# noegroup/bgflow

Measured on AMD Instinct MI355X. Metric: flow samples/s (fwd+log|detJ|) at batch 2^20, higher is better.
Workload: dtype f32 (split-f16 conditioner GEMMs: hi+lo f16 operand pairs, f32 accumulate)

## Files before the change

### bgflow_amd/csrc/bgk_fused2.hip

```cpp
#include "bgk_common.h"
#include "bgk_fused2.h"

#ifndef BGK_V2_SAVE
#define BGK_V2_SAVE 0
#endif
#if BGK_V2_SAVE
#include "bgk_mfma_h2.h"
#include "bgk_rqs_vjp.h"
#define coupling_rqs_dense_h2v2_kernel coupling_rqs_dense_h2v2_train_kernel
#endif
#ifndef BGK_V2_BF16
#define BGK_V2_BF16 0
#endif
#if BGK_V2_BF16
#define coupling_rqs_dense_h2v2_kernel coupling_rqs_dense_h2v2_bf16_kernel
typedef short s16x8 __attribute__((ext_vector_type(8)));
#endif
#ifndef BGK_V2_AFFTRAIN
#define BGK_V2_AFFTRAIN 0
#endif
#if BGK_V2_AFFTRAIN
#define coupling_affine_dense_v2_kernel coupling_affine_dense_v2_train_kernel
#endif
constexpr int NPROD = BGK_V2_BF16 ? 1 : 3;
// ... 150 lines not shown
    template <int E0, int E1>
    __device__ __forceinline__ void events() {
        if constexpr (E0 < E1) {
            event<E0>();
            events<E0 + 1, E1>();
        }
    }
    template <int HK, int NH>
    __device__ __forceinline__ void hook() {
        constexpr int e0 = (HK * NEV) / NH, e1 = ((HK + 1) * NEV) / NH;
        if constexpr (e0 < e1) events<e0, e1>();
    }
};
struct NoLive {
    template <int HK, int NH> __device__ __forceinline__ void hook() {}
};

template <int NT>
struct LiveTM {
    static constexpr int LPT = KS + 1;
    static constexpr int NLS = LPT * NT;
    static constexpr int EPT = 3 * KS + 1;
    static constexpr int NEV = EPT * NT;
    static constexpr int tile_of(int i) { return NT == 4 ? (i == 0 ? 1 : (i == 1 ? 3 : (i == 2 ? 0 : 2))) : (i == 0 ? 1 : 0); }
    f32x16 (&out)[4];
    const BFrag& b;
    const uint4* W;
    unsigned voff;
    TFrag (&ring)[RD];
    __amdgpu_buffer_rsrc_t rs;

    template <int BLK>
    __device__ __forceinline__ u32x4 blk() {
        return __builtin_amdgcn_raw_buffer_load_b128(rs, voff + ((BLK * 1024) & 4095), (BLK * 1024) & ~4095, 0);
    }
    template <int L>
    __device__ __forceinline__ void load() {
        if constexpr (L < NLS) {
            constexpr int s = L % LPT, m = tile_of(L / LPT);
            if constexpr (s < KS) {
                ring[L % RD].hi = blk<(s * 4 + m) * 2>();
                ring[L % RD].lo = blk<(s * 4 + m) * 2 + 1>();
            } else {
                ring[L % RD].hi = blk<KS * 4 * 2 + m>();
            }
        }
    }
    template <int L0, int L1>
    __device__ __forceinline__ void loads() {
        if constexpr (L0 < L1) { load<L0>(); loads<L0 + 1, L1>(); }
    }
    __device__ __forceinline__ void start() {
        __builtin_amdgcn_sched_barrier(0);
        rs = __builtin_amdgcn_make_buffer_rsrc((void*)W, 0, 0x7fffffff, 0x00020000);
        loads<0, RD>();
        __builtin_amdgcn_sched_barrier(0);
    }
    template <int E>
    __device__ __forceinline__ void event() {
        __builtin_amdgcn_sched_barrier(0);
        if constexpr (E < NEV) {
            constexpr int i = E / EPT, e = E % EPT, m = tile_of(i);
            if constexpr (e < 3 * KS) {
                constexpr int s = e / 3, p = e % 3, L = i * LPT + s;
                const TFrag& f = ring[L % RD];
                const h16x8 a = __builtin_bit_cast(h16x8, p == 0 ? f.lo : f.hi);
                const h16x8 bb = p == 1 ? b.lo[s] : b.hi[s];
                if constexpr (s == 0 && p == 0) {
                    const f32x16 z = {0.f, 0.f, 0.f, 0.f, 0.f, 0.f, 0.f, 0.f, 0.f, 0.f, 0.f, 0.f, 0.f, 0.f, 0.f, 0.f};
                    out[m] = __builtin_amdgcn_mfma_f32_32x32x16_f16(a, bb, z, 0, 0, 0);
                } else {
                    out[m] = __builtin_amdgcn_mfma_f32_32x32x16_f16(a, bb, out[m], 0, 0, 0);
                }
                if constexpr (p == 2) load<L + RD>();
            } else {
                constexpr int L = i * LPT + KS;
                const h16x8 one2 = {(_Float16)1.0f, (_Float16)1.0f, 0, 0, 0, 0, 0, 0};
                out[m] = __builtin_amdgcn_mfma_f32_32x32x16_f16(__builtin_bit_cast(h16x8, ring[L % RD].hi), one2, out[m], 0, 0, 0);
                load<L + RD>();
            }
        }
        __builtin_amdgcn_sched_barrier(0);
    }
    template <int E0, int E1>
    __device__ __forceinline__ void events() {
        if constexpr (E0 < E1) {
            event<E0>();
            events<E0 + 1, E1>();
        }
    }
    template <int HK, int NH>
    __device__ __forceinline__ void hook() {
        constexpr int e0 = (HK * NEV) / NH, e1 = ((HK + 1) * NEV) / NH;
        if constexpr (e0 < e1) events<e0, e1>();
    }
};

template <class G, int BASE, int NH>
struct Hooks {
    G& g;
    template <int I> __device__ __forceinline__ void at() { g.template hook<BASE + I, NH>(); }
};

template <int ACT, int T, int P, class H>
__device__ __forceinline__ void act_split_pair(H& hk, const f32x16& t, float c, BFrag& bf) {
    constexpr int r = 2 * P;
    float a0, a1;
    if constexpr (ACT == 2) {
        a0 = t[r] * c; a1 = t[r + 1] * c;
        hk.template at<3 * P>();
        a0 = a0 > 0.0f ? a0 : 0.0f; a1 = a1 > 0.0f ? a1 : 0.0f;
        hk.template at<3 * P + 1>();
    } else {
        constexpr float kk = ACT == 1 ? -1.44269504088896341f : 2.88539008177792681f;
        const float ck = c * kk, rc = 1.0f / c;
        const float e0 = __builtin_amdgcn_exp2f(t[r] * ck), e1 = __builtin_amdgcn_exp2f(t[r + 1] * ck);
        hk.template at<3 * P>();
        if constexpr (ACT == 1) {
            const float q0 = __builtin_amdgcn_rcpf(__builtin_fmaf(e0, rc, rc)), q1 = __builtin_amdgcn_rcpf(__builtin_fmaf(e1, rc, rc));
            a0 = t[r] * q0; a1 = t[r + 1] * q1;
        } else {
            const float q0 = __builtin_amdgcn_rcpf(1.0f + e0), q1 = __builtin_amdgcn_rcpf(1.0f + e1);
            a0 = 1.0f - 2.0f * q0; a1 = 1.0f - 2.0f * q1;
        }
        hk.template at<3 * P + 1>();
    }
    constexpr int s = 2 * T + (r >> 3), e = r & 7;
#if BGK_V2_BF16
    typedef __bf16 bf2v __attribute__((ext_vector_type(2)));
    typedef float f2v __attribute__((ext_vector_type(2)));
    typedef _Float16 h2v __attribute__((ext_vector_type(2)));
    const bf2v pb = __builtin_convertvector((f2v){a0, a1}, bf2v);
    const h2v ph = __builtin_bit_cast(h2v, pb);
    bf.hi[s][e] = ph[0]; bf.hi[s][e + 1] = ph[1];
#else
    unsigned uh, ul;
    asm("v_cvt_pk_f16_f32 %0, %1, %2" : "=v"(uh) : "v"(a0), "v"(a1));
    asm("v_fma_mixlo_f16 %0, %1, -1.0, %2 op_sel:[0,0,0] op_sel_hi:[1,0,0]" : "=v"(ul) : "v"(uh), "v"(a0));
    asm("v_fma_mixhi_f16 %0, %1, -1.0, %2 op_sel:[1,0,0] op_sel_hi:[1,0,0]" : "+v"(ul) : "v"(uh), "v"(a1));
    typedef _Float16 h2v __attribute__((ext_vector_type(2)));
    const h2v ph = __builtin_bit_cast(h2v, uh), pl = __builtin_bit_cast(h2v, ul);
    bf.hi[s][e] = ph[0]; bf.hi[s][e + 1] = ph[1];
    bf.lo[s][e] = pl[0]; bf.lo[s][e + 1] = pl[1];
#endif
    hk.template at<3 * P + 2>();
}
template <int ACT, int T, class H>
__device__ __forceinline__ void act_split_tile(H hk, const f32x16& t, float c, BFrag& bf) {
    act_split_pair<ACT, T, 0>(hk, t, c, bf); act_split_pair<ACT, T, 1>(hk, t, c, bf);
    act_split_pair<ACT, T, 2>(hk, t, c, bf); act_split_pair<ACT, T, 3>(hk, t, c, bf);
    act_split_pair<ACT, T, 4>(hk, t, c, bf); act_split_pair<ACT, T, 5>(hk, t, c, bf);
    act_split_pair<ACT, T, 6>(hk, t, c, bf); act_split_pair<ACT, T, 7>(hk, t, c, bf);
}

struct SpK { float kL, kz, c2; };

__device__ __forceinline__ float fdiv_hw(float n, float d) {
    const float r = __builtin_amdgcn_rcpf(d);
    const float q = n * r;
    return __builtin_fmaf(__builtin_fmaf(-d, q, n), r, q);
}

template <bool KARG> struct ScSrc;
template <> struct ScSrc<true> {
    kargs_t ka;
    __device__ __forceinline__ ScSrc(const V2Args&) { ka = (kargs_t)__builtin_amdgcn_kernarg_segment_ptr(); asm volatile("" : "+s"(ka)); }
    __device__ __forceinline__ const __attribute__((address_space(4))) SpC& get() const { return ka->sc; }
};
template <> struct ScSrc<false> {
    const V2Args& a;
    __device__ __forceinline__ ScSrc(const V2Args& a_) : a(a_) {}
    __device__ __forceinline__ const SpC& get() const { return a.sc; }
};

template <int INV, class H>
__device__ __forceinline__ float rqs_fast(H hk, float x, const float (&va)[KB], const float (&vb)[KB], const float* ps, int pst, bool circ,
                                          const V2Args& a, const SpK& k, float* lad, int* bin, int* oob) {
    const ScSrc<(BGK_V2_KARG == 2 ? INV != 0 : BGK_V2_KARG != 0)> scs(a);
#define SC scs.get()
    *oob = (x < SC.left) | (x > SC.right);
    x = __builtin_amdgcn_fmed3f(x, SC.left, SC.right);
    float mA = __builtin_fmaxf(__builtin_fmaxf(va[0], va[1]), va[2]);
    mA = __builtin_fmaxf(__builtin_fmaxf(mA, va[3]), va[4]);
    mA = __builtin_fmaxf(__builtin_fmaxf(mA, va[5]), va[6]);
    mA = __builtin_fmaxf(mA, va[7]);
    const float nmA = -(mA * k.kL);
    hk.template at<0>();
    float E[KB];
    E[0] = __builtin_amdgcn_exp2f(__builtin_fmaf(va[0], k.kL, nmA));
    E[1] = __builtin_amdgcn_exp2f(__builtin_fmaf(va[1], k.kL, nmA));
    E[2] = __builtin_amdgcn_exp2f(__builtin_fmaf(va[2], k.kL, nmA));
    hk.template at<1>();
    E[3] = __builtin_amdgcn_exp2f(__builtin_fmaf(va[3], k.kL, nmA));
    E[4] = __builtin_amdgcn_exp2f(__builtin_fmaf(va[4], k.kL, nmA));
    E[5] = __builtin_amdgcn_exp2f(__builtin_fmaf(va[5], k.kL, nmA));
    hk.template at<2>();
    E[6] = __builtin_amdgcn_exp2f(__builtin_fmaf(va[6], k.kL, nmA));
    E[7] = __builtin_amdgcn_exp2f(__builtin_fmaf(va[7], k.kL, nmA));
    E[1] += E[0]; E[2] += E[1];
    hk.template at<3>();
    E[3] += E[2]; E[4] += E[3]; E[5] += E[4]; E[6] += E[5]; E[7] += E[6];
    hk.template at<4>();
    const float gA = SC.sa.gnum * bgk_rcp_refined(E[7]);
    float kn[7];
    kn[0] = __builtin_fmaf(E[0], gA, SC.sa.kc[0]);
    kn[1] = __builtin_fmaf(E[1], gA, SC.sa.kc[1]);
    hk.template at<5>();
    kn[2] = __builtin_fmaf(E[2], gA, SC.sa.kc[2]);
    kn[3] = __builtin_fmaf(E[3], gA, SC.sa.kc[3]);
    kn[4] = __builtin_fmaf(E[4], gA, SC.sa.kc[4]);
    kn[5] = __builtin_fmaf(E[5], gA, SC.sa.kc[5]);
    kn[6] = __builtin_fmaf(E[6], gA, SC.sa.kc[6]);
    hk.template at<6>();
    float low_a = SC.sa.low, high_a = SC.sa.high;
    asm volatile("" : "+s"(low_a), "+s"(high_a));
#pragma unroll
    for (int i = 0; i < 7; ++i) asm volatile("" : "+v"(kn[i]));
    const bool g3 = x >= kn[3];
    hk.template at<7>();
    float w0 = g3 ? kn[3] : low_a, w1 = g3 ? kn[4] : kn[0], w2 = g3 ? kn[5] : kn[1], w3 = g3 ? kn[6] : kn[2];
    hk.template at<8>();
    float w4 = g3 ? high_a : kn[3];
    const bool gm = x >= w2;
    const float v0 = gm ? w2 : w0, v1 = gm ? w3 : w1, v2 = gm ? w4 : w2;
    hk.template at<9>();
    const bool gl = x >= v1;
    const float lo = gl ? v1 : v0, hi = gl ? v2 : v1;
    float idxf = g3 ? 4.0f : 0.0f;
    hk.template at<10>();
    idxf += gm ? 2.0f : 0.0f;
    idxf += gl ? 1.0f : 0.0f;
    const int idx = (int)idxf;
    *bin = idx;
    hk.template at<11>();
    const int j1 = circ ? ((idx + 1) & 7) : (idx + 1);
    const float s_lo = ps[idx * pst], s_hi = ps[j1 * pst];
    const float A_i = hi - lo;
    float mB = __builtin_fmaxf(__builtin_fmaxf(vb[0], vb[1]), vb[2]);
    hk.template at<12>();
    mB = __builtin_fmaxf(__builtin_fmaxf(mB, vb[3]), vb[4]);
    mB = __builtin_fmaxf(__builtin_fmaxf(mB, vb[5]), vb[6]);
    mB = __builtin_fmaxf(mB, vb[7]);
    const float nmB = -(mB * k.kL);
    float F[KB];
    F[0] = __builtin_amdgcn_exp2f(__builtin_fmaf(vb[0], k.kL, nmB));
    hk.template at<13>();
    F[1] = __builtin_amdgcn_exp2f(__builtin_fmaf(vb[1], k.kL, nmB));
    F[2] = __builtin_amdgcn_exp2f(__builtin_fmaf(vb[2], k.kL, nmB));
    F[3] = __builtin_amdgcn_exp2f(__builtin_fmaf(vb[3], k.kL, nmB));
    hk.template at<14>();
    F[4] = __builtin_amdgcn_exp2f(__builtin_fmaf(vb[4], k.kL, nmB));
    F[5] = __builtin_amdgcn_exp2f(__builtin_fmaf(vb[5], k.kL, nmB));
    F[6] = __builtin_amdgcn_exp2f(__builtin_fmaf(vb[6], k.kL, nmB));
    hk.template at<15>();
    F[7] = __builtin_amdgcn_exp2f(__builtin_fmaf(vb[7], k.kL, nmB));
    F[1] += F[0]; F[2] += F[1]; F[3] += F[2];
    hk.template at<16>();
    F[4] += F[3]; F[5] += F[4]; F[6] += F[5]; F[7] += F[6];
    const float rB = __builtin_amdgcn_rcpf(F[7]);
    hk.template at<17>();
    const float gB = SC.sb.gnum * __builtin_fmaf(__builtin_fmaf(-F[7], rB, 1.0f), rB, rB);
    const float f0 = g3 ? F[3] : 0.0f, f1 = g3 ? F[4] : F[0], f2 = g3 ? F[5] : F[1];
    hk.template at<18>();
    const float f3 = g3 ? F[6] : F[2], f4 = g3 ? F[7] : F[3];
    const float u0 = gm ? f2 : f0, u1 = gm ? f3 : f1, u2 = gm ? f4 : f2;
    hk.template at<19>();
    const float Flo = gl ? u1 : u0;
    float Fhi = gl ? u2 : u1;
    hk.template at<20>();
    const float cb = __builtin_fmaf(idxf, SC.sb.dstep, SC.sb.low);
    hk.template at<21>();
    const float b_i = __builtin_fmaf(Flo, gB, cb);
    float b_ip1 = __builtin_fmaf(Fhi, gB, cb + SC.sb.dstep);
    float top_b = SC.sb.high;
    asm volatile("" : "+s"(top_b));
    b_ip1 = (g3 && gm && gl) ? top_b : b_ip1;
    const float B_i = b_ip1 - b_i;
    const float z0 = s_lo * k.kz;
    hk.template at<22>();
    const float ez0 = __builtin_amdgcn_exp2f(z0);
    float lg0 = __builtin_amdgcn_logf(1.0f + ez0);
    asm volatile("" : "+v"(lg0));
    const float sm0 = ez0 * __builtin_fmaf(ez0, -0.5f, 1.0f) * 1.44269504088896341f;
    hk.template at<23>();
    float l0 = (ez0 < 2.44140625e-4f ? sm0 : lg0) * SC.kout;
    asm volatile("" : "+v"(l0));
    l0 = z0 > 28.8539008177792681f ? s_lo * k.c2 : l0;
    const float d_i = SC.min_d + l0;
    const float z1 = s_hi * k.kz;
    hk.template at<24>();
    const float ez1 = __builtin_amdgcn_exp2f(z1);
    float lg1 = __builtin_amdgcn_logf(1.0f + ez1);
    asm volatile("" : "+v"(lg1));
    const float sm1 = ez1 * __builtin_fmaf(ez1, -0.5f, 1.0f) * 1.44269504088896341f;
    hk.template at<25>();
    float l1 = (ez1 < 2.44140625e-4f ? sm1 : lg1) * SC.kout;
    asm volatile("" : "+v"(l1));
    l1 = z1 > 28.8539008177792681f ? s_hi * k.c2 : l1;
    const float d_ip1 = SC.min_d + l1;
    float cw_i, W_i, ch_i, H_i;
    if (INV) { cw_i = lo; W_i = A_i; ch_i = b_i; H_i = B_i; }
    else { ch_i = lo; H_i = A_i; cw_i = b_i; W_i = B_i; }
    hk.template at<26>();
    const float delta = fdiv_hw(H_i, W_i);
    const float S = d_i + d_ip1 - 2.0f * delta;
    hk.template at<27>();
// ... 170 lines not shown
    s_y[valid ? j * a.ys + dim : 32 * a.ys + j] = o;
    oob_local += (valid && j < rows) ? oob : 0;
    bins[IT] = bin;
    lad = valid ? lad : 0.0f;
    float l0 = lad, l1 = lad;
    asm volatile("s_nop 1\n\tv_permlane32_swap_b32 %0, %1" : "+v"(l0), "+v"(l1));
    run += l0;
    run += l1;
}

template <int INV, int NT>
__device__ __forceinline__ void chunk_piped_reg(const V2Args& a, const SpK& k, float* s_p, float* s_y, int c, int hh, int j, int rows,
                                                float& run, int& oob_local, int (&bins)[3], f32x16 (&h)[4], const BFrag& bf,
                                                TFrag (&ring)[RD], unsigned voff) {
    LiveTM<NT> g{h, bf, a.A2 + (size_t)(c + 1) * GBLK * 64, voff, ring};
    g.start();
    slab_to_lds(h, s_p, hh, j);
    __builtin_amdgcn_sched_barrier(0);
    spline_slot_reg<INV, 0, 3 * EH>(g, a, k, h[0], s_p, s_y, c, DPC, hh, j, rows, run, oob_local, bins);
    spline_slot_reg<INV, 1, 3 * EH>(g, a, k, h[2], s_p, s_y, c, DPC, hh, j, rows, run, oob_local, bins);
    spline_slot_reg<INV, 2, 3 * EH>(g, a, k, h[2], s_p, s_y, c, DPC, hh, j, rows, run, oob_local, bins);
}

typedef const __attribute__((address_space(1))) void* gvp_t;
typedef __attribute__((address_space(3))) void* lvp_t;
__device__ __forceinline__ void dma_tile32(float* dst, const float* __restrict__ src, int n, int valid, int lane) {
    for (int c = 0; c < n; c += 256) {
        const int e = c + lane * 4;
        if (e + 3 < valid) __builtin_amdgcn_global_load_lds((gvp_t)(src + e), (lvp_t)(dst + c), 16, 0, 0);
    }
    if (valid & 3) {
        const int edge = valid & ~3;
        if (lane < (valid & 3)) __builtin_amdgcn_global_load_lds((gvp_t)(src + edge + lane), (lvp_t)(dst + edge), 4, 0, 0);
    }
}

__device__ __forceinline__ void v2_sincos2pi(float x, float* s, float* c) {
    const float f = __builtin_amdgcn_fractf(x);
    *s = __builtin_amdgcn_sinf(f);
    *c = __builtin_amdgcn_cosf(f);
}

struct StageTiles { int d_c, periodic, nfs, ys, stage, y_dma, d; uint32_t magic_d; int rows, lane; };

__device__ __forceinline__ void stage_issue(const StageTiles& t, const CondSegs& cs, int64_t b0, const float* y_t, float* s_p, float* s_y) {
    if (t.y_dma) dma_tile32(s_y, y_t, 32 * t.d, t.rows * t.d, t.lane);
    if (t.stage == 1) dma_tile32(s_p, cs.ptr[0] + b0 * cs.ld[0], 32 * t.d_c, t.rows * t.d_c, t.lane);
    else if (t.stage == 2) dma_tile32(s_p + 32 * t.nfs, cs.ptr[0] + b0 * cs.ld[0], 32 * t.d_c, t.rows * t.d_c, t.lane);
}

#ifndef BGK_V2_SB
#define BGK_V2_SB 8
#endif
template <class KA>
__device__ __forceinline__ void stage_finish(const StageTiles& t, const CondSegs& cs, int64_t b0, const float* y_t, int ldy32,
                                             float* s_p, float* s_y, float y_fill) {
    constexpr int SB = BGK_V2_SB;
    const int lane = t.lane, rows = t.rows, d = t.d, nfs = t.nfs, n_y = 32 * t.d;
    if (!t.y_dma) {
        for (int base = 0; base < n_y; base += 64 * SB) {
            float vy[SB];
#pragma unroll
            for (int u = 0; u < SB; ++u) {
                const int i = base + u * 64 + lane;
                const int r = (int)(__umul24((unsigned)i, t.magic_d) >> 20), c = i - (int)__umul24((unsigned)r, (unsigned)d);
                vy[u] = (i < n_y && r < rows) ? y_t[(int)__umul24((unsigned)r, (unsigned)ldy32) + c] : y_fill;
            }
#pragma unroll
            for (int u = 0; u < SB; ++u) {
                const int i = base + u * 64 + lane;
                const int r = (int)(__umul24((unsigned)i, t.magic_d) >> 20), c = i - (int)__umul24((unsigned)r, (unsigned)d);
                if (i < n_y) s_y[(int)__umul24((unsigned)r, (unsigned)t.ys) + c] = vy[u];
            }
        }
    }
    if (t.stage == 0) {
        typedef const __attribute__((address_space(4))) KA* ka_t;
        const ka_t kseg = (ka_t)__builtin_amdgcn_kernarg_segment_ptr();
        for (int sg = 0; sg < cs.n; ++sg) {
            const float* cond_t = kseg->cs.ptr[sg] + b0 * kseg->cs.ld[sg];
            const int ldc32 = (int)kseg->cs.ld[sg], w_c = kseg->cs.w[sg], n_c = 32 * w_c, col0 = kseg->cs.off[sg];
            const uint32_t magic_c = kseg->cs.magic[sg];
            for (int base = 0; base < n_c; base += 64 * SB) {
                float vc[SB];
#pragma unroll
                for (int u = 0; u < SB; ++u) {
                    const int i = base + u * 64 + lane;
                    const int r = (int)(__umul24((unsigned)i, magic_c) >> 20), c = i - (int)__umul24((unsigned)r, (unsigned)w_c);
                    vc[u] = (i < n_c && r < rows) ? cond_t[(int)__umul24((unsigned)r, (unsigned)ldc32) + c] : 0.0f;
                }
#pragma unroll
                for (int u = 0; u < SB; ++u) {
                    const int i = base + u * 64 + lane;
                    const int r = (int)(__umul24((unsigned)i, magic_c) >> 20), c = i - (int)__umul24((unsigned)r, (unsigned)w_c);
                    if (i < n_c) {
                        float* f = s_p + (int)__umul24((unsigned)r, (unsigned)nfs) + col0 + c;
                        if (t.periodic) {
                            float sv, cv;
                            v2_sincos2pi(vc[u], &sv, &cv);
                            f[0] = cv;
                            f[t.d_c] = sv;
                        } else {
                            f[0] = vc[u];
                        }
                    }
                }
            }
        }
    }
    asm volatile("s_waitcnt vmcnt(0)" ::: "memory");
    __builtin_amdgcn_fence(__ATOMIC_ACQ_REL, "wavefront");
    __builtin_amdgcn_wave_barrier();
    if (t.stage == 2) {
        const float* raw = s_p + 32 * nfs;
        const uint32_t magic_c = cs.magic[0];
        for (int i = lane; i < 32 * t.d_c; i += 64) {
            const int r = (int)(__umul24((unsigned)i, magic_c) >> 20), c = i - (int)__umul24((unsigned)r, (unsigned)t.d_c);
            float sv, cv;
            v2_sincos2pi(raw[i], &sv, &cv);
            float* f = s_p + (int)__umul24((unsigned)r, (unsigned)nfs) + c;
            f[0] = cv;
            f[t.d_c] = sv;
        }
    }
    if (t.stage != 1) {
        __builtin_amdgcn_fence(__ATOMIC_ACQ_REL, "wavefront");
        __builtin_amdgcn_wave_barrier();
    }
}

__device__ __forceinline__ void store_tile32(float* out_t, int ldo32, const float* s_y, int ys, int d, uint32_t magic_d, int rows, int lane, int lin) {
    const int n = rows * d;
    if (lin) {
        for (int i = lane * 4; i + 3 < n; i += 256) *reinterpret_cast<float4*>(out_t + i) = *reinterpret_cast<const float4*>(s_y + i);
        if (lane < (n & 3)) out_t[(n & ~3) + lane] = s_y[(n & ~3) + lane];
    } else {
        for (int i = lane; i < n; i += 64) {
            const int r = (int)(__umul24((unsigned)i, magic_d) >> 20), cc = i - (int)__umul24((unsigned)r, (unsigned)d);
            out_t[(int)__umul24((unsigned)r, (unsigned)ldo32) + cc] = s_y[(int)__umul24((unsigned)r, (unsigned)ys) + cc];
        }
    }
}

struct L0Frag { uint4 v[4][2]; };
__device__ __forceinline__ void l0_request(L0Frag& f, const uint4* A0, int s, int lane) {
#pragma unroll
    for (int m = 0; m < 4; ++m) {
        f.v[m][0] = A0[((s * 4 + m) * 2 + 0) * 64 + lane];
#if !BGK_V2_BF16
        f.v[m][1] = A0[((s * 4 + m) * 2 + 1) * 64 + lane];
#endif
    }
}
__device__ __forceinline__ void l0_step(f32x16 (&h)[4], const L0Frag& fr, const float* f, bool last, int rel0) {
    float v[8];
#pragma unroll
    for (int e = 0; e < 8; ++e) v[e] = f[e];
    if (last) {
#pragma unroll
        for (int e = 0; e < 8; ++e) v[e] = rel0 + e == 0 ? 1.0f : (rel0 + e > 0 ? 0.0f : v[e]);
    }
#if BGK_V2_BF16
    s16x8 bb;
#pragma unroll
    for (int e = 0; e < 8; ++e) bb[e] = __builtin_bit_cast(short, (__bf16)v[e]);
#pragma unroll
    for (int m = 0; m < 4; ++m)
        h[m] = __builtin_amdgcn_mfma_f32_32x32x16_bf16(__builtin_bit_cast(s16x8, fr.v[m][0]), bb, h[m], 0, 0, 0);
#else
    h16x8 bhi, blo;
#pragma unroll
    for (int e = 0; e < 8; ++e) {
        const float c = v[e];
        const _Float16 hv = (_Float16)c;
        bhi[e] = hv;
        blo[e] = (_Float16)(c - (float)hv);
    }
#pragma unroll
    for (int m = 0; m < 4; ++m) h[m] = __builtin_amdgcn_mfma_f32_32x32x16_f16(__builtin_bit_cast(h16x8, fr.v[m][1]), bhi, h[m], 0, 0, 0);
#pragma unroll
    for (int m = 0; m < 4; ++m) h[m] = __builtin_amdgcn_mfma_f32_32x32x16_f16(__builtin_bit_cast(h16x8, fr.v[m][0]), blo, h[m], 0, 0, 0);
#pragma unroll
    for (int m = 0; m < 4; ++m) h[m] = __builtin_amdgcn_mfma_f32_32x32x16_f16(__builtin_bit_cast(h16x8, fr.v[m][0]), bhi, h[m], 0, 0, 0);
#endif
}

template <int ACT, int INV, bool SAVEP = true, bool REGP = false>
__global__ __launch_bounds__(FTHREADS, 2) void coupling_rqs_dense_h2v2_kernel(V2Args a) {
    static_assert(!REGP || (!BGK_V2_SAVE && !BGK_V2_BF16), "row order 2 belongs to the split-f16 inference instance");
    if (a.cs_dev) { a.c0 = a.cs_dev[1]; a.c1 = a.cs_dev[3]; a.c2 = a.cs_dev[5]; }
    asm volatile("s_setreg_imm32_b32 hwreg(HW_REG_MODE, 23, 1), 1");
    extern __shared__ __attribute__((aligned(16))) float smem[];
    const int wave = REGP ? __builtin_amdgcn_readfirstlane((int)(threadIdx.x >> 6)) : (int)(threadIdx.x >> 6);
    float* s_p = smem + (size_t)wave * a.lds_per_wave;
    float* s_y = s_p + (REGP ? a.p_floats : 128 * ST);
    const int d = a.d;
    const int64_t n_tiles = (a.B + 31) / 32;
    const int64_t tile = (int64_t)blockIdx.x * FW + wave;
    if (tile >= n_tiles) return;
    const SpK k{a.c2 * 1.44269504088896341f, a.c2 * a.sc.beta * 1.44269504088896341f, a.c2};
    const int n_in = a.periodic ? 2 * a.d_c : a.d_c;
    const int ldy32 = (int)a.ldy, ldo32 = (int)a.ldo;
    const int n_y = 32 * d;

  {
    const int lane = (int)threadIdx.x & 63, j = lane & 31, hh = lane >> 5;
    const unsigned voff = (unsigned)lane * 16u;
    const int64_t b0 = tile * 32;
    const int rows = (int)((a.B - b0) < 32 ? (a.B - b0) : 32);
    const float* y_t = a.y + b0 * a.ldy;
    float* out_t = a.out + b0 * a.ldo;
    V2_TS(0);

    const int nfs = a.nfs, ys = a.ys;
    const StageTiles stg{a.d_c, a.periodic, nfs, ys, a.stage, a.y_dma, d, a.magic_d, rows, lane};
    stage_issue(stg, a.cs, b0, y_t, s_p, s_y);
    f32x16 h[4], acc[4];
    TFrag ring[RD];
    BFrag bf;
    L0Frag fa, fb;
    l0_request(fa, a.A0, 0, lane);
    Live<4> g1{acc, bf, a.A1, voff, ring};
    g1.start();
    V2_TS(12);
    stage_finish<V2Args>(stg, a.cs, b0, y_t, ldy32, s_p, s_y, 0.5f);
    V2_TS(1);

#pragma unroll
    for (int m = 0; m < 4; ++m)
#pragma unroll
        for (int r = 0; r < 16; ++r) h[m][r] = 0.0f;
    {
        const float* frow = s_p + j * nfs + 8 * hh;
        const int rel0 = 16 * (a.S0 - 1) + 8 * hh - n_in;
        for (int s = 0; s < a.S0; s += 2) {
            if (s + 1 < a.S0) l0_request(fb, a.A0, s + 1, lane);
            l0_step(h, fa, frow + 16 * s, s + 1 == a.S0, rel0);
            if (s + 1 < a.S0) {
                if (s + 2 < a.S0) l0_request(fa, a.A0, s + 2, lane);
                l0_step(h, fb, frow + 16 * (s + 1), s + 2 == a.S0, rel0);
            }
        }
    }

    V2_TS(2);
    {
        Live<4>& g = g1;
#if BGK_V2_SAVE
#pragma unroll
        for (int m = 0; m < 4; ++m)
#pragma unroll
            for (int r = 0; r < 16; ++r) h[m][r] *= a.c0;
        h2_store_rows128(h, a.z0, s_p, b0, rows, lane);
        const float c0_act = 1.0f;
#else
        const float c0_act = a.c0;
#endif
        NoLive none;
        act_split_tile<ACT, 0>(Hooks<NoLive, 0, 1>{none}, h[0], c0_act, bf);
        __builtin_amdgcn_sched_barrier(0);
        V2_TS(14);
        act_split_tile<ACT, 1>(Hooks<Live<4>, 0, 100>{g}, h[1], c0_act, bf);
        act_split_tile<ACT, 2>(Hooks<Live<4>, 24, 100>{g}, h[2], c0_act, bf);
        act_split_tile<ACT, 3>(Hooks<Live<4>, 48, 100>{g}, h[3], c0_act, bf);
        __builtin_amdgcn_sched_barrier(0);
        V2_TS(15);
        g.template events<(72 * Live<4>::NEV) / 100, Live<4>::NEV>();
    }

    V2_TS(3);
    float run = 0.0f;
    int oob_local = 0;
    {
        Live<4> g{h, bf, a.A2, voff, ring};
        g.start();
#if BGK_V2_SAVE
#pragma unroll
        for (int m = 0; m < 4; ++m)
#pragma unroll
            for (int r = 0; r < 16; ++r) acc[m][r] *= a.c1;
        h2_store_rows128(acc, a.z1, s_p, b0, rows, lane);
        const float c1_act = 1.0f;
#else
        const float c1_act = a.c1;
#endif
        NoLive none;
        act_split_tile<ACT, 0>(Hooks<NoLive, 0, 1>{none}, acc[0], c1_act, bf);
        __builtin_amdgcn_sched_barrier(0);
        act_split_tile<ACT, 1>(Hooks<Live<4>, 0, 100>{g}, acc[1], c1_act, bf);
        act_split_tile<ACT, 2>(Hooks<Live<4>, 24, 100>{g}, acc[2], c1_act, bf);
        act_split_tile<ACT, 3>(Hooks<Live<4>, 48, 100>{g}, acc[3], c1_act, bf);
        __builtin_amdgcn_sched_barrier(0);
        g.template events<(72 * Live<4>::NEV) / 100, Live<4>::NEV>();
    }
    V2_TS(4);
    for (int c = 0; c < a.n_chunks; ++c) {
        int bins[3] = {0, 0, 0};
        const int nd = (d - c * DPC) < DPC ? (d - c * DPC) : DPC;
        if constexpr (REGP) {
            if (c + 2 < a.n_chunks || (c + 2 == a.n_chunks && a.last_tiles > 2)) {
                chunk_piped_reg<INV, 4>(a, k, s_p, s_y, c, hh, j, rows, run, oob_local, bins, h, bf, ring, voff);
            } else if (c + 2 == a.n_chunks) {
                chunk_piped_reg<INV, 2>(a, k, s_p, s_y, c, hh, j, rows, run, oob_local, bins, h, bf, ring, voff);
            } else {
                NoLive none;
                slab_to_lds(h, s_p, hh, j);
                spline_slot_reg<INV, 0, 1>(none, a, k, h[0], s_p, s_y, c, nd, hh, j, rows, run, oob_local, bins);
                if (nd > 2) spline_slot_reg<INV, 1, 1>(none, a, k, h[2], s_p, s_y, c, nd, hh, j, rows, run, oob_local, bins);
                if (nd > 4) spline_slot_reg<INV, 2, 1>(none, a, k, h[2], s_p, s_y, c, nd, hh, j, rows, run, oob_local, bins);
            }
        } else
        if (c + 2 < a.n_chunks || (c + 2 == a.n_chunks && a.last_tiles > 2)) {
            chunk_piped<INV, 4, SAVEP>(a, k, s_p, s_y, c, hh, j, rows, run, oob_local, bins, h, bf, ring, voff, b0);
        } else if (c + 2 == a.n_chunks) {
            chunk_piped<INV, 2, SAVEP>(a, k, s_p, s_y, c, hh, j, rows, run, oob_local, bins, h, bf, ring, voff, b0);
        } else {
            NoLive none;
            chunk_to_lds(h, s_p, hh, j);
#if BGK_V2_SAVE
            if constexpr (SAVEP) save_chunk_params(a, s_p, c, lane, b0, rows);
#endif
            spline_slot<INV, 0, 1>(none, a, k, s_p, s_y, c, nd, hh, j, rows, run, oob_local, bins);
            if (nd > 2) spline_slot<INV, 1, 1>(none, a, k, s_p, s_y, c, nd, hh, j, rows, run, oob_local, bins);
            if (nd > 4) spline_slot<INV, 2, 1>(none, a, k, s_p, s_y, c, nd, hh, j, rows, run, oob_local, bins);
        }
#if BGK_V2_TS
        V2_TS(5 + c);
#else
        if (a.bin_idx) {
#pragma unroll
            for (int it = 0; it < 3; ++it) {
                const int q = 2 * it + hh;
                if (q < nd && j < rows) a.bin_idx[(b0 + j) * d + c * DPC + q] = bins[it];
            }
        }
#endif
        __builtin_amdgcn_fence(__ATOMIC_ACQ_REL, "wavefront");
        __builtin_amdgcn_wave_barrier();
    }
    int lane_e = lane;
    if constexpr (REGP) {
        int zero = 0;
        asm volatile("" : "+v"(zero));
        lane_e = (int)__builtin_amdgcn_mbcnt_hi(~0u, __builtin_amdgcn_mbcnt_lo(~0u, (unsigned)zero));
    }
    if ((lane_e >> 5) == 0 && (lane_e & 31) < rows) {
        if (a.accumulate) a.dlogp[b0 + (lane_e & 31)] += run; else a.dlogp[b0 + (lane_e & 31)] = run;
    }
    store_tile32(out_t, ldo32, s_y, ys, d, a.magic_d, rows, lane_e, a.out_lin);
    if (a.oob_count && __builtin_amdgcn_ballot_w64(oob_local != 0)) {
        for (int off = 32; off > 0; off >>= 1) oob_local += __shfl_xor(oob_local, off);
        if (lane_e == 0) atomicAdd(a.oob_count, oob_local);
    }
    V2_TS(5 + a.n_chunks);
  }
}

struct TilePlan { int nfs, ys, stage, y_dma, out_lin; };
TilePlan plan_tiles(const CondSegs& cs, int d_c, int periodic, const float* y, int64_t ldy, const float* out, int64_t ldo, int d, int tile_floats) {
    const int n_in = periodic ? 2 * d_c : d_c;
    const auto dma_ok = [](const float* p, int64_t ld, int w) { return ld == w && ((uintptr_t)p & 15) == 0 && (w & 7) != 0; };
    TilePlan t;
    t.y_dma = dma_ok(y, ldy, d) ? 1 : 0;
    t.ys = t.y_dma ? d : (d | 1);
    t.out_lin = (t.y_dma && ldo == d && ((uintptr_t)out & 15) == 0) ? 1 : 0;
    const bool c_dma = cs.n == 1 && dma_ok(cs.ptr[0], cs.ld[0], d_c);
    t.stage = (c_dma && !periodic) ? 1 : ((c_dma && periodic && 32 * ((n_in | 1) + d_c) <= tile_floats) ? 2 : 0);
    t.nfs = t.stage == 1 ? d_c : (n_in | 1);
    return t;
}

SetK make_set(double low, double high, double min_bin, int K) {
    SetK s;
    const double span = high - low, scale = 1.0 - min_bin * K;
    s.gnum = (float)((double)(float)span * (double)(float)scale);
    s.low = (float)low; s.high = (float)high;
    s.dstep = (float)((double)(float)span * (double)(float)min_bin);
    for (int k = 0; k < 7; ++k) s.kc[k] = (float)((double)(float)low + (double)(float)span * (double)(float)min_bin * (k + 1));
    return s;
}

uint32_t magic_div(int d) { return (uint32_t)(((1u << 20) + (uint32_t)d - 1) / (uint32_t)d); }

bool make_cond_segs(CondSegs& cs, const float* cond, int64_t ldc, int d_c, const BgkCondSegs* segs) {
    for (int i = 0; i < BGK_MAX_COND; ++i) { cs.ptr[i] = nullptr; cs.ld[i] = 0; cs.w[i] = 0; cs.off[i] = 0; cs.magic[i] = 0; }
    if (!segs || segs->n <= 1) {
        const float* p = segs && segs->n == 1 ? segs->ptr[0] : cond;
        const int64_t ld = segs && segs->n == 1 ? segs->ld[0] : ldc;
        if (!p || d_c <= 0 || ld >= (1 << 24)) return false;
        cs.n = 1; cs.ptr[0] = p; cs.ld[0] = ld; cs.w[0] = d_c; cs.magic[0] = magic_div(d_c);
        return true;
    }
    if (segs->n > BGK_MAX_COND) return false;
    int off = 0;
    for (int i = 0; i < segs->n; ++i) {
        if (!segs->ptr[i] || segs->w[i] <= 0 || segs->ld[i] < segs->w[i] || segs->ld[i] >= (1 << 24)) return false;
        cs.ptr[i] = segs->ptr[i]; cs.ld[i] = segs->ld[i]; cs.w[i] = segs->w[i]; cs.off[i] = off; cs.magic[i] = magic_div(segs->w[i]);
        off += segs->w[i];
    }
    cs.n = segs->n;
    return off == d_c;
}


#if !BGK_V2_SAVE && !BGK_V2_BF16
struct AffV2Net { const uint4* A0; const uint4* A1; const uint4* A1b; const uint4* A2; float c0, c1, c1b, c2;
#if BGK_V2_AFFTRAIN
                  const float* cs;
                  float* z0; float* z1;
#endif
};
struct AffV2Args {
    CondSegs cs; int d_c; int periodic; int S0;
    AffV2Net shift, scale; int has_shift, has_scale;
    const float* log_alpha; int preserve_volume, is_circular, inverse;
    const float* y; int64_t ldy; int64_t B; int d;
    float* out; int64_t ldo; float* dlogp; int accumulate;
    uint32_t magic_d;
    int lds_tile, lds_per_wave;
    int nfs, ys, stage, y_dma, out_lin;
#if BGK_V2_AFFTRAIN
    float* mu_out; float* s_out; int64_t ldms;
    int slab;
    int zt;
#endif
};

#if BGK_V2_AFFTRAIN
template <int NT>
__device__ __forceinline__ void aff_store_tiles(const f32x16 (&t)[4], float* dst, int pitch, float* slab, int64_t b0, int rows, int lane) {
    const int j = lane & 31, hh = lane >> 5;
    const __amdgpu_buffer_rsrc_t rs = __builtin_amdgcn_make_buffer_rsrc((void*)(dst + b0 * pitch), 0, rows * pitch * 4, 0x00020000);
#pragma unroll
    for (int m = 0; m < NT; ++m)
#pragma unroll
        for (int half = 0; half < 2; ++half) {
            if ((j >> 4) == half) {
#pragma unroll
                for (int q = 0; q < 4; ++q)
                    *reinterpret_cast<float4*>(slab + (j & 15) * 32 + 4 * ((2 * q + hh) ^ (j & 7))) =
                        make_float4(t[m][4 * q], t[m][4 * q + 1], t[m][4 * q + 2], t[m][4 * q + 3]);
            }
            __builtin_amdgcn_fence(__ATOMIC_ACQ_REL, "wavefront");
            __builtin_amdgcn_wave_barrier();
#pragma unroll
            for (int it = 0; it < 2; ++it) {
                const int i = it * 64 + lane, r = i >> 3, p = i & 7;
                const float4 v = *reinterpret_cast<const float4*>(slab + r * 32 + 4 * (p ^ (r & 7)));
                __builtin_amdgcn_raw_buffer_store_b128(__builtin_bit_cast(u32x4, v), rs, ((16 * half + r) * pitch + 32 * m + 4 * p) * 4, 0, 0);
            }
            __builtin_amdgcn_fence(__ATOMIC_ACQ_REL, "wavefront");
            __builtin_amdgcn_wave_barrier();
        }
}
struct AffSave { float* slab; int64_t b0; int rows, lane, zt; };
#endif

__device__ __forceinline__ void aff_layer0(const AffV2Net& n, int S0, const float* s_p, int nfs, int n_in, int lane, int j, int hh,
                                           f32x16 (&X)[4], L0Frag& fa, bool requested) {
    L0Frag fb;
    if (!requested) l0_request(fa, n.A0, 0, lane);
#pragma unroll
    for (int m = 0; m < 4; ++m)
#pragma unroll
        for (int r = 0; r < 16; ++r) X[m][r] = 0.0f;
    const float* frow = s_p + j * nfs + 8 * hh;
    const int rel0 = 16 * (S0 - 1) + 8 * hh - n_in;
    for (int s = 0; s < S0; s += 2) {
        if (s + 1 < S0) l0_request(fb, n.A0, s + 1, lane);
        l0_step(X, fa, frow + 16 * s, s + 1 == S0, rel0);
        if (s + 1 < S0) {
            if (s + 2 < S0) l0_request(fa, n.A0, s + 2, lane);
            l0_step(X, fb, frow + 16 * (s + 1), s + 2 == S0, rel0);
        }
    }
}

#if BGK_V2_AFFTRAIN
#define AFF_SAVE_PARAMS , float* zdst, const AffSave& sv
#define AFF_SAVE_Z(X) do { _Pragma("unroll") for (int m_ = 0; m_ < 4; ++m_) _Pragma("unroll") for (int r_ = 0; r_ < 16; ++r_) X[m_][r_] *= c; \
                           if (sv.zt == 2) aff_store_tiles<2>(X, zdst, 64, sv.slab, sv.b0, sv.rows, sv.lane); \
                           else aff_store_tiles<4>(X, zdst, 128, sv.slab, sv.b0, sv.rows, sv.lane); \
                           c = 1.0f; } while (0)
#else
#define AFF_SAVE_PARAMS
#define AFF_SAVE_Z(X) do { } while (0)
#endif
template <int ACT>
__device__ __forceinline__ void aff_hidden(const uint4* A, float c, f32x16 (&X)[4], f32x16 (&Y)[4], BFrag& bf, TFrag (&ring)[RD], unsigned voff AFF_SAVE_PARAMS) {
    NoLive none;
    Live<4> g{Y, bf, A, voff, ring};
    g.start();
    AFF_SAVE_Z(X);
    act_split_tile<ACT, 0>(Hooks<NoLive, 0, 1>{none}, X[0], c, bf);
    __builtin_amdgcn_sched_barrier(0);
    act_split_tile<ACT, 1>(Hooks<Live<4>, 0, 100>{g}, X[1], c, bf);
    act_split_tile<ACT, 2>(Hooks<Live<4>, 24, 100>{g}, X[2], c, bf);
    act_split_tile<ACT, 3>(Hooks<Live<4>, 48, 100>{g}, X[3], c, bf);
    __builtin_amdgcn_sched_barrier(0);
    g.template events<(72 * Live<4>::NEV) / 100, Live<4>::NEV>();
// ... 591 lines not shown
```

Measured before the change: 137.6 million.

## Software-pipeline activation split across pairs and triple-buffer layer-0 weight loads

Adds a carried activation/split path that defers the final fma_mixhi and fragment writes of each pair into the next pair's iteration, interleaved with the live MFMA hooks, to hide the VALU dependency latency. Layer-0 GEMM now uses three rotating weight-fragment buffers with deeper prefetch, starts the g1 pipeline after staging, and folds the zero-init into the first MFMA via a zero accumulator. The accumulate flag is read from kernarg via scalar pointer in the REGP path. These raise register pressure and change scheduling of the inference instance only.

```diff
diff --git a/bgflow_amd/csrc/bgk_fused2.hip b/bgflow_amd/csrc/bgk_fused2.hip
--- a/bgflow_amd/csrc/bgk_fused2.hip
+++ b/bgflow_amd/csrc/bgk_fused2.hip
@@ -326,6 +326,56 @@
     act_split_pair<ACT, T, 4>(hk, t, c, bf); act_split_pair<ACT, T, 5>(hk, t, c, bf);
     act_split_pair<ACT, T, 6>(hk, t, c, bf); act_split_pair<ACT, T, 7>(hk, t, c, bf);
 }
+
+#define BGK_V2_SPLIT_CARRY (!BGK_V2_SAVE && !BGK_V2_BF16)
+#if !BGK_V2_BF16
+struct SplitCarry { unsigned uh, ul; float a1; };
+template <int I>
+__device__ __forceinline__ void split_carry_finish(BFrag& bf, SplitCarry& pc) {
+    constexpr int T = 1 + I / 8, r = 2 * (I % 8), s = 2 * T + (r >> 3), e = r & 7;
+    asm("v_fma_mixhi_f16 %0, %1, -1.0, %2 op_sel:[1,0,0] op_sel_hi:[1,0,0]" : "+v"(pc.ul) : "v"(pc.uh), "v"(pc.a1));
+    typedef _Float16 h2v __attribute__((ext_vector_type(2)));
+    const h2v ph = __builtin_bit_cast(h2v, pc.uh), pl = __builtin_bit_cast(h2v, pc.ul);
+    bf.hi[s][e] = ph[0]; bf.hi[s][e + 1] = ph[1];
+    bf.lo[s][e] = pl[0]; bf.lo[s][e + 1] = pl[1];
+}
+template <int ACT, int I, class G>
+__device__ __forceinline__ void act_split_carried(G& g, const f32x16 (&X)[4], float c, BFrag& bf, SplitCarry& pc) {
+    if constexpr (I < 24) {
+        constexpr int T = 1 + I / 8, r = 2 * (I % 8);
+        const f32x16& t = X[T];
+        float a0, a1;
+        if constexpr (ACT == 2) {
+            a0 = t[r] * c; a1 = t[r + 1] * c;
+            if constexpr (I > 0) split_carry_finish<I - 1>(bf, pc);
+            g.template hook<3 * I, 100>();
+            a0 = a0 > 0.0f ? a0 : 0.0f; a1 = a1 > 0.0f ? a1 : 0.0f;
+        } else {
+            constexpr float kk = ACT == 1 ? -1.44269504088896341f : 2.88539008177792681f;
+            const float ck = c * kk, rc = 1.0f / c;
+            const float x0 = t[r] * ck, x1 = t[r + 1] * ck;
+            if constexpr (I > 0) split_carry_finish<I - 1>(bf, pc);
+            const float e0 = __builtin_amdgcn_exp2f(x0), e1 = __builtin_amdgcn_exp2f(x1);
+            g.template hook<3 * I, 100>();
+            if constexpr (ACT == 1) {
+                const float q0 = __builtin_amdgcn_rcpf(__builtin_fmaf(e0, rc, rc)), q1 = __builtin_amdgcn_rcpf(__builtin_fmaf(e1, rc, rc));
+                a0 = t[r] * q0; a1 = t[r + 1] * q1;
+            } else {
+                const float q0 = __builtin_amdgcn_rcpf(1.0f + e0), q1 = __builtin_amdgcn_rcpf(1.0f + e1);
+                a0 = 1.0f - 2.0f * q0; a1 = 1.0f - 2.0f * q1;
+            }
+        }
+        asm("v_cvt_pk_f16_f32 %0, %1, %2" : "=v"(pc.uh) : "v"(a0), "v"(a1));
+        g.template hook<3 * I + 1, 100>();
+        asm("v_fma_mixlo_f16 %0, %1, -1.0, %2 op_sel:[0,0,0] op_sel_hi:[1,0,0]" : "=v"(pc.ul) : "v"(pc.uh), "v"(a0));
+        pc.a1 = a1;
+        g.template hook<3 * I + 2, 100>();
+        act_split_carried<ACT, I + 1>(g, X, c, bf, pc);
+    } else {
+        split_carry_finish<23>(bf, pc);
+    }
+}
+#endif
 
 struct SpK { float kL, kz, c2; };
 
@@ -802,7 +852,9 @@
 #endif
     }
 }
+template <bool FIRST = false>
 __device__ __forceinline__ void l0_step(f32x16 (&h)[4], const L0Frag& fr, const float* f, bool last, int rel0) {
+    const f32x16 z = {0.f, 0.f, 0.f, 0.f, 0.f, 0.f, 0.f, 0.f, 0.f, 0.f, 0.f, 0.f, 0.f, 0.f, 0.f, 0.f};
     float v[8];
 #pragma unroll
     for (int e = 0; e < 8; ++e) v[e] = f[e];
@@ -816,7 +868,7 @@
     for (int e = 0; e < 8; ++e) bb[e] = __builtin_bit_cast(short, (__bf16)v[e]);
 #pragma unroll
     for (int m = 0; m < 4; ++m)
-        h[m] = __builtin_amdgcn_mfma_f32_32x32x16_bf16(__builtin_bit_cast(s16x8, fr.v[m][0]), bb, h[m], 0, 0, 0);
+        h[m] = __builtin_amdgcn_mfma_f32_32x32x16_bf16(__builtin_bit_cast(s16x8, fr.v[m][0]), bb, FIRST ? z : h[m], 0, 0, 0);
 #else
     h16x8 bhi, blo;
 #pragma unroll
@@ -827,12 +879,75 @@
         blo[e] = (_Float16)(c - (float)hv);
     }
 #pragma unroll
-    for (int m = 0; m < 4; ++m) h[m] = __builtin_amdgcn_mfma_f32_32x32x16_f16(__builtin_bit_cast(h16x8, fr.v[m][1]), bhi, h[m], 0, 0, 0);
+    for (int m = 0; m < 4; ++m) h[m] = __builtin_amdgcn_mfma_f32_32x32x16_f16(__builtin_bit_cast(h16x8, fr.v[m][1]), bhi, FIRST ? z : h[m], 0, 0, 0);
 #pragma unroll
     for (int m = 0; m < 4; ++m) h[m] = __builtin_amdgcn_mfma_f32_32x32x16_f16(__builtin_bit_cast(h16x8, fr.v[m][0]), blo, h[m], 0, 0, 0);
 #pragma unroll
     for (int m = 0; m < 4; ++m) h[m] = __builtin_amdgcn_mfma_f32_32x32x16_f16(__builtin_bit_cast(h16x8, fr.v[m][0]), bhi, h[m], 0, 0, 0);
 #endif
+}
+
+template <class G>
+__device__ __forceinline__ void v2_head(const V2Args& a, const StageTiles& stg, G& g1, f32x16 (&h)[4], int64_t b0, const float* y_t,
+                                        int ldy32, float* s_p, float* s_y, int n_in, int lane, int j, int hh) {
+    const int d = a.d, S0 = a.S0;
+    L0Frag f0, f1, f2;
+    l0_request(f0, a.A0, 0, lane);
+    if (S0 > 1) l0_request(f1, a.A0, 1, lane);
+    if (S0 > 2) l0_request(f2, a.A0, 2, lane);
+    V2_TS(12);
+    stage_finish<V2Args>(stg, a.cs, b0, y_t, ldy32, s_p, s_y, 0.5f);
+    g1.start();
+    V2_TS(1);
+    const float* frow = s_p + j * stg.nfs + 8 * hh;
+    const int rel0 = 16 * (S0 - 1) + 8 * hh - n_in;
+    l0_step<true>(h, f0, frow, S0 == 1, rel0);
+    if (S0 > 1) {
+        if (S0 > 3) l0_request(f0, a.A0, 3, lane);
+        l0_step(h, f1, frow + 16, S0 == 2, rel0);
+    }
+    if (S0 > 2) {
+        if (S0 > 4) l0_request(f1, a.A0, 4, lane);
+        l0_step(h, f2, frow + 32, S0 == 3, rel0);
+    }
+    for (int s = 3; s < S0; s += 3) {
+        if (s + 2 < S0) l0_request(f2, a.A0, s + 2, lane);
+        l0_step(h, f0, frow + 16 * s, s + 1 == S0, rel0);
+        if (s + 1 < S0) {
+            if (s + 3 < S0) l0_request(f0, a.A0, s + 3, lane);
+            l0_step(h, f1, frow + 16 * (s + 1), s + 2 == S0, rel0);
+        }
+        if (s + 2 < S0) {
+            if (s + 4 < S0) l0_request(f1, a.A0, s + 4, lane);
+            l0_step(h, f2, frow + 16 * (s + 2), s + 3 == S0, rel0);
+        }
+    }
+}
+
+template <class G>
+__device__ __forceinline__ void v2_head_pair(const V2Args& a, const StageTiles& stg, G& g1, f32x16 (&h)[4], int64_t b0, const float* y_t,
+                                             int ldy32, float* s_p, float* s_y, int n_in, int lane, int j, int hh) {
+    const int d = a.d;
+    L0Frag fa, fb;
+    l0_request(fa, a.A0, 0, lane);
+    g1.start();
+    V2_TS(12);
+    stage_finish<V2Args>(stg, a.cs, b0, y_t, ldy32, s_p, s_y, 0.5f);
+    V2_TS(1);
+#pragma unroll
+    for (int m = 0; m < 4; ++m)
+#pragma unroll
+        for (int r = 0; r < 16; ++r) h[m][r] = 0.0f;
+    const float* frow = s_p + j * stg.nfs + 8 * hh;
+    const int rel0 = 16 * (a.S0 - 1) + 8 * hh - n_in;
+    for (int s = 0; s < a.S0; s += 2) {
+        if (s + 1 < a.S0) l0_request(fb, a.A0, s + 1, lane);
+        l0_step(h, fa, frow + 16 * s, s + 1 == a.S0, rel0);
+        if (s + 1 < a.S0) {
+            if (s + 2 < a.S0) l0_request(fa, a.A0, s + 2, lane);
+            l0_step(h, fb, frow + 16 * (s + 1), s + 2 == a.S0, rel0);
+        }
+    }
 }
 
 template <int ACT, int INV, bool SAVEP = true, bool REGP = false>
@@ -868,30 +983,9 @@
     f32x16 h[4], acc[4];
     TFrag ring[RD];
     BFrag bf;
-    L0Frag fa, fb;
-    l0_request(fa, a.A0, 0, lane);
     Live<4> g1{acc, bf, a.A1, voff, ring};
-    g1.start();
-    V2_TS(12);
-    stage_finish<V2Args>(stg, a.cs, b0, y_t, ldy32, s_p, s_y, 0.5f);
-    V2_TS(1);
-
-#pragma unroll
-    for (int m = 0; m < 4; ++m)
-#pragma unroll
-        for (int r = 0; r < 16; ++r) h[m][r] = 0.0f;
-    {
-        const float* frow = s_p + j * nfs + 8 * hh;
-        const int rel0 = 16 * (a.S0 - 1) + 8 * hh - n_in;
-        for (int s = 0; s < a.S0; s += 2) {
-            if (s + 1 < a.S0) l0_request(fb, a.A0, s + 1, lane);
-            l0_step(h, fa, frow + 16 * s, s + 1 == a.S0, rel0);
-            if (s + 1 < a.S0) {
-                if (s + 2 < a.S0) l0_request(fa, a.A0, s + 2, lane);
-                l0_step(h, fb, frow + 16 * (s + 1), s + 2 == a.S0, rel0);
-            }
-        }
-    }
+    if constexpr (BGK_V2_SAVE || BGK_V2_BF16) v2_head_pair(a, stg, g1, h, b0, y_t, ldy32, s_p, s_y, n_in, lane, j, hh);
+    else v2_head(a, stg, g1, h, b0, y_t, ldy32, s_p, s_y, n_in, lane, j, hh);
 
     V2_TS(2);
     {
@@ -910,9 +1004,13 @@
         act_split_tile<ACT, 0>(Hooks<NoLive, 0, 1>{none}, h[0], c0_act, bf);
         __builtin_amdgcn_sched_barrier(0);
         V2_TS(14);
+#if BGK_V2_SPLIT_CARRY
+        { SplitCarry pc; act_split_carried<ACT, 0>(g, h, c0_act, bf, pc); }
+#else
         act_split_tile<ACT, 1>(Hooks<Live<4>, 0, 100>{g}, h[1], c0_act, bf);
         act_split_tile<ACT, 2>(Hooks<Live<4>, 24, 100>{g}, h[2], c0_act, bf);
         act_split_tile<ACT, 3>(Hooks<Live<4>, 48, 100>{g}, h[3], c0_act, bf);
+#endif
         __builtin_amdgcn_sched_barrier(0);
         V2_TS(15);
         g.template events<(72 * Live<4>::NEV) / 100, Live<4>::NEV>();
@@ -937,9 +1035,13 @@
         NoLive none;
         act_split_tile<ACT, 0>(Hooks<NoLive, 0, 1>{none}, acc[0], c1_act, bf);
         __builtin_amdgcn_sched_barrier(0);
+#if BGK_V2_SPLIT_CARRY
+        { SplitCarry pc; act_split_carried<ACT, 0>(g, acc, c1_act, bf, pc); }
+#else
         act_split_tile<ACT, 1>(Hooks<Live<4>, 0, 100>{g}, acc[1], c1_act, bf);
         act_split_tile<ACT, 2>(Hooks<Live<4>, 24, 100>{g}, acc[2], c1_act, bf);
         act_split_tile<ACT, 3>(Hooks<Live<4>, 48, 100>{g}, acc[3], c1_act, bf);
+#endif
         __builtin_amdgcn_sched_barrier(0);
         g.template events<(72 * Live<4>::NEV) / 100, Live<4>::NEV>();
     }
@@ -994,8 +1096,9 @@
         asm volatile("" : "+v"(zero));
         lane_e = (int)__builtin_amdgcn_mbcnt_hi(~0u, __builtin_amdgcn_mbcnt_lo(~0u, (unsigned)zero));
     }
+    const int accumulate = REGP ? ScSrc<true>(a).ka->accumulate : a.accumulate;
     if ((lane_e >> 5) == 0 && (lane_e & 31) < rows) {
-        if (a.accumulate) a.dlogp[b0 + (lane_e & 31)] += run; else a.dlogp[b0 + (lane_e & 31)] = run;
+        if (accumulate) a.dlogp[b0 + (lane_e & 31)] += run; else a.dlogp[b0 + (lane_e & 31)] = run;
     }
     store_tile32(out_t, ldo32, s_y, ys, d, a.magic_d, rows, lane_e, a.out_lin);
     if (a.oob_count && __builtin_amdgcn_ballot_w64(oob_local != 0)) {
```

After: 138.6 million (median of 6 runs). About the same (+0.7%).
